# arangesh/Ground-Plane-Polling

Measured on AMD Instinct MI355X. Metric: images/sec end-to-end (resnet50, 1k planes, 1242x375), higher is better.
Workload: dtype f16x3

## Files before the change

ground-plane-polling_amd/csrc/decode.hip:

```cpp

#include <hip/hip_runtime.h>
#include <stdint.h>
#include <limits.h>

#include <atomic>
#include <mutex>
#include <vector>

#include "gpp.h"

namespace {

constexpr int kCounterStride = 4096;
constexpr int kHeaderBytes = 64 * kCounterStride;
constexpr int kKeptCountWord = 1;
constexpr int kKeptKeysOffset = 1024;

__device__ __forceinline__ float cephes_expf(float x)
{
    x = fminf(fmaxf(x, -88.3762626647949f), 88.3762626647949f);
    float fx = floorf(x * 1.44269504088896341f + 0.5f);
    x = (x - fx * 0.693359375f) - fx * -2.12194440e-4f;
    const float z = x * x;
    float y = 1.9875691500e-4f;
// ... 767 lines not shown
{
    compact_pixels(bitmap, T, B, max_rows, rows, counts, flag, or_flag);
}

struct CompactJob { uint32_t* bitmap; int32_t* rows; int32_t* counts; int32_t* flag; const int32_t* or_flag; };
__global__ __launch_bounds__(kCompactThreads) void compact_pixels_pair_kernel(const CompactJob a, const CompactJob b, const LevelTable T, int B, int max_rows)
{
    const CompactJob& j = blockIdx.x == 0 ? a : b;
    compact_pixels(j.bitmap, T, B, max_rows, j.rows, j.counts, j.flag, j.or_flag);
}

__global__ __launch_bounds__(256) void mark_candidate_pixels_kernel(const float* __restrict__ cls, int64_t n_anchors, int nba, float thr,
                                                                    const LevelTable T, int B, int total_words, uint32_t* __restrict__ marks)
{
    __shared__ unsigned long long hit[4];
    const int lane = threadIdx.x & 63, wave = threadIdx.x >> 6;
    const int64_t gbit0 = (int64_t)blockIdx.x * 256 + wave * 64;
    const int word0 = (int)(gbit0 >> 5);
    if (lane == 0) hit[wave] = 0;
    __syncthreads();
    for (int i = 0; i < nba; ++i) {
        const int j = i * 64 + lane, q = j / nba, k = j - q * nba;
        const int word = word0 + (q >> 5);
        if (word >= total_words) continue;
        int l = 0;
        for (int t = 1; t < T.n_levels; ++t) l = word >= T.word_begin[t] ? t : l;
        const int64_t bit = gbit0 + q - ((int64_t)T.word_begin[l] << 5);
        const int pix = T.pix[l];
        if (bit >= (int64_t)B * pix) continue;
        const int b = (int)(bit / pix), p = (int)(bit - (int64_t)b * pix);
        const float4* src = (const float4*)(cls + ((int64_t)b * n_anchors + (int64_t)(T.pix_begin[l] + p) * nba + k) * 8);
        const float4 v0 = src[0], v1 = src[1];
        const float lg[8] = {v0.x, v0.y, v0.z, v0.w, v1.x, v1.y, v1.z, v1.w};
        Folded f;
        if (is_candidate(lg, thr, f)) atomicOr(&hit[wave], 1ull << q);
    }
    __syncthreads();
    const unsigned long long mask = hit[wave];
    if (lane == 0 && word0 < total_words) marks[word0] = (uint32_t)mask;
    if (lane == 32 && word0 + 1 < total_words) marks[word0 + 1] = (uint32_t)(mask >> 32);
}

__global__ __launch_bounds__(256) void dilate_radii_kernel(const uint32_t* __restrict__ marks, const LevelTable T, int B, int total_words,
                                                           uint32_t* __restrict__ radius1, uint32_t* __restrict__ radius2,
                                                           uint32_t* __restrict__ radius3)
{
    const int64_t gbit = (int64_t)blockIdx.x * 256 + threadIdx.x;
    const int word = (int)(gbit >> 5);
    if (word >= total_words) return;
    int l = 0;
    for (int q = 1; q < T.n_levels; ++q) l = word >= T.word_begin[q] ? q : l;
    const int64_t bit = gbit - ((int64_t)T.word_begin[l] << 5);
    const int pix = T.pix[l], W = T.width[l], H = pix / W;
    bool on1 = false, on2 = false, on3 = false;
    if (bit < (int64_t)B * pix) {
        const int b = (int)(bit / pix), p = (int)(bit - (int64_t)b * pix);
        const int y = p / W, x = p - y * W;
        const uint32_t* words = marks + T.word_begin[l];
        for (int dy = -3; dy <= 3; ++dy) {
            const int yy = y + dy;
            if (yy < 0 || yy >= H) continue;
            for (int dx = -3; dx <= 3; ++dx) {
                const int xx = x + dx;
                if (xx < 0 || xx >= W) continue;
                const int64_t nb = (int64_t)b * pix + yy * W + xx;
                const bool v = (words[nb >> 5] >> (nb & 31)) & 1u;
                const int r = max(abs(dy), abs(dx));
                on3 |= v;
                on2 |= v && r <= 2;
                on1 |= v && r <= 1;
            }
        }
    }
    const unsigned long long m1 = __ballot(on1), m2 = __ballot(on2), m3 = __ballot(on3);
    const int lane = threadIdx.x & 63;
    if (lane == 0 || lane == 32) {
        const int sh = lane;
        radius1[word] = (uint32_t)(m1 >> sh);
        radius2[word] = (uint32_t)(m2 >> sh);
        radius3[word] = (uint32_t)(m3 >> sh);
    }
}

__global__ __launch_bounds__(kCompactThreads) void deep_stats_kernel(const uint32_t* __restrict__ marks, const uint32_t* __restrict__ radius1,
                                                                     const uint32_t* __restrict__ radius2, int total_words, int max_rows,
                                                                     int tower_max_rows, int deep_max_rows, int32_t* __restrict__ stats)
{
    __shared__ int sums[3][kCompactThreads / 64];
    const int tid = threadIdx.x, lane = tid & 63, wave = tid >> 6;
    int n[3] = {0, 0, 0};
    for (int w = tid; w < total_words; w += kCompactThreads) {
        n[0] += __popc(marks[w]);
        n[1] += __popc(radius1[w]);
        n[2] += __popc(radius2[w]);
    }
#pragma unroll
    for (int k = 0; k < 3; ++k) {
#pragma unroll
        for (int s = 32; s >= 1; s >>= 1) n[k] += __shfl_down(n[k], s, 64);
        if (lane == 0) sums[k][wave] = n[k];
    }
    __syncthreads();
    if (tid == 0) {
        int t[3] = {0, 0, 0};
        for (int q = 0; q < kCompactThreads / 64; ++q) { t[0] += sums[0][q]; t[1] += sums[1][q]; t[2] += sums[2][q]; }
        const int f3 = (t[0] > max_rows || t[1] > tower_max_rows) ? 1 : 0;
        stats[0] = t[0];
        stats[1] = t[1];
        stats[2] = f3;
        stats[3] = (f3 || t[2] > deep_max_rows) ? 1 : 0;
    }
}

std::mutex g_deep_mutex;
std::vector<gpp_deep_list_desc> g_deep_descs;
std::vector<char> g_deep_held;

}

extern "C" int gpp_detect_pixel_lists(const gpp_pixel_list_desc* host_desc, void* stream)
{
    if (!host_desc) return GPP_ERR_BAD_ARG;
    const gpp_pixel_list_desc& d = *host_desc;
    if (d.B < 0 || d.B > kMaxBatch || d.n_anchors <= 0 || d.n_anchors > kMaxAnchors || d.num_base_anchors <= 0 || d.max_rows < 0 ||
        d.n_levels < 1 || d.n_levels > GPP_MAX_GROUPS || (d.lists_per_image != 1 && d.lists_per_image != 4) || d.reserved != 0 || d.reserved2 != 0)
        return GPP_ERR_BAD_ARG;
    if (d.B == 0) return GPP_OK;
    if (!d.workspace || !d.bitmap || !d.rows || !d.counts || !d.flag) return GPP_ERR_BAD_ARG;
    if (((uintptr_t)d.workspace & 15) || (((uintptr_t)d.bitmap | (uintptr_t)d.rows | (uintptr_t)d.counts | (uintptr_t)d.flag) & 3)) return GPP_ERR_ALIGN;
    const bool dilate = d.dilated_bitmap || d.dilated_rows || d.dilated_counts || d.dilated_flag;
    if (dilate && (!d.dilated_bitmap || !d.dilated_rows || !d.dilated_counts || !d.dilated_flag || d.dilated_max_rows < 0)) return GPP_ERR_BAD_ARG;
    if (((uintptr_t)d.dilated_bitmap | (uintptr_t)d.dilated_rows | (uintptr_t)d.dilated_counts | (uintptr_t)d.dilated_flag) & 3) return GPP_ERR_ALIGN;
    const int lists = d.B * d.lists_per_image;
    if (lists > 64) return GPP_ERR_UNSUPPORTED;
    LevelTable T;
    T.n_levels = d.n_levels;
    int64_t pixels = 0, words = 0;
    for (int l = 0; l < GPP_MAX_GROUPS; ++l) {
        const int pix = l < d.n_levels ? d.level_pixels[l] : 0;
        if (l < d.n_levels && pix <= 0) return GPP_ERR_BAD_ARG;
        if ((int64_t)d.B * (pixels + pix) >= (1LL << 31)) return GPP_ERR_UNSUPPORTED;
        T.pix[l] = pix;
        T.pix_begin[l] = (int)pixels;
        T.word_begin[l] = (int)words;
        T.list_begin[l] = (int)((int64_t)d.B * pixels);
        T.width[l] = (dilate && l < d.n_levels) ? d.level_width[l] : 0;
        if (dilate && l < d.n_levels && (T.width[l] <= 0 || pix % T.width[l] != 0)) return GPP_ERR_BAD_ARG;
        pixels += pix;
        words += ((int64_t)d.B * pix + 31) / 32;
    }
    if (pixels * d.num_base_anchors != d.n_anchors) return GPP_ERR_BAD_ARG;
    hipStream_t st = (hipStream_t)stream;
    const unsigned char* ws = (const unsigned char*)d.workspace;
    const int32_t* cnt = (const int32_t*)ws;
    const unsigned long long* keys = (const unsigned long long*)(ws + kHeaderBytes);
    mark_pixels_kernel<<<dim3(16, (unsigned)lists), 256, 0, st>>>(keys, cnt, pow2_ceil(d.n_anchors), d.n_anchors, d.num_base_anchors,
                                                                   d.lists_per_image, T, d.bitmap);
    if (dilate) {
        const int64_t pairs = (words + 1) / 2;
        dilate_pixels_kernel<<<dim3((unsigned)((pairs * 64 + 255) / 256)), 256, 0, st>>>(d.bitmap, T, d.B, (int)words, d.dilated_bitmap);
    }
    compact_pixels_kernel<<<1, kCompactThreads, 0, st>>>(d.bitmap, T, d.B, d.max_rows, d.rows, d.counts, d.flag, nullptr);
    if (dilate)
        compact_pixels_kernel<<<1, kCompactThreads, 0, st>>>(d.dilated_bitmap, T, d.B, d.dilated_max_rows, d.dilated_rows, d.dilated_counts,
                                                             d.dilated_flag, d.flag);
    const hipError_t e = hipGetLastError();
    return e == hipSuccess ? GPP_OK : (int)e;
}

namespace {

int deep_lists_table(const gpp_deep_list_desc& d, LevelTable& T, int64_t& words)
{
    if (d.B < 0 || d.B > kMaxBatch || d.n_anchors <= 0 || d.n_anchors > kMaxAnchors || d.num_base_anchors <= 0 || d.num_base_anchors > 64 ||
        d.max_rows < 0 || d.tower_max_rows < 0 || d.deep_max_rows < 0 || d.n_levels < 1 || d.n_levels > GPP_MAX_GROUPS || d.reserved != 0 ||
        !(d.score_thr == d.score_thr))
        return GPP_ERR_BAD_ARG;
    const bool layer1 = d.rows1 || d.counts1 || d.flag1;
    if (d.B > 0 && (!d.cls_logits || !d.marks || !d.radius1 || !d.radius2 || !d.radius3 || !d.rows2 || !d.counts2 || !d.flag2 || !d.stats ||
                    (layer1 && (!d.rows1 || !d.counts1 || !d.flag1))))
        return GPP_ERR_BAD_ARG;
    if (((uintptr_t)d.cls_logits & 15) || (((uintptr_t)d.marks | (uintptr_t)d.radius1 | (uintptr_t)d.radius2 | (uintptr_t)d.radius3 | (uintptr_t)d.rows2 |
          (uintptr_t)d.counts2 | (uintptr_t)d.flag2 | (uintptr_t)d.rows1 | (uintptr_t)d.counts1 | (uintptr_t)d.flag1 | (uintptr_t)d.stats) & 3))
        return GPP_ERR_ALIGN;
    T.n_levels = d.n_levels;
    int64_t pixels = 0;
    words = 0;
    for (int l = 0; l < GPP_MAX_GROUPS; ++l) {
        const int pix = l < d.n_levels ? d.level_pixels[l] : 0;
        if (l < d.n_levels && pix <= 0) return GPP_ERR_BAD_ARG;
        if ((int64_t)d.B * (pixels + pix) >= (1LL << 31)) return GPP_ERR_UNSUPPORTED;
        T.pix[l] = pix;
        T.pix_begin[l] = (int)pixels;
        T.word_begin[l] = (int)words;
        T.list_begin[l] = (int)((int64_t)d.B * pixels);
        T.width[l] = l < d.n_levels ? d.level_width[l] : 0;
        if (l < d.n_levels && (T.width[l] <= 0 || pix % T.width[l] != 0)) return GPP_ERR_BAD_ARG;
        pixels += pix;
        words += ((int64_t)d.B * pix + 31) / 32;
    }
    if (pixels * d.num_base_anchors != d.n_anchors) return GPP_ERR_BAD_ARG;
    return GPP_OK;
}

}

extern "C" int gpp_detect_deep_lists(const gpp_deep_list_desc* host_desc, void* stream)
{
    if (!host_desc) return GPP_ERR_BAD_ARG;
    const gpp_deep_list_desc& d = *host_desc;
    LevelTable T;
    int64_t words = 0;
    const int rc = deep_lists_table(d, T, words);
    if (rc != GPP_OK) return rc;
    if (d.B == 0) return GPP_OK;
    hipStream_t st = (hipStream_t)stream;
    const unsigned blocks = (unsigned)(((words + 1) / 2 * 64 + 255) / 256);
    mark_candidate_pixels_kernel<<<dim3(blocks), 256, 0, st>>>(d.cls_logits, d.n_anchors, d.num_base_anchors, d.score_thr, T, d.B, (int)words, d.marks);
    dilate_radii_kernel<<<dim3(blocks), 256, 0, st>>>(d.marks, T, d.B, (int)words, d.radius1, d.radius2, d.radius3);
    deep_stats_kernel<<<1, kCompactThreads, 0, st>>>(d.marks, d.radius1, d.radius2, (int)words, d.max_rows, d.tower_max_rows, d.deep_max_rows, d.stats);
    const CompactJob layer2 = {d.radius2, d.rows2, d.counts2, d.flag2, d.stats + 2}, layer1 = {d.radius3, d.rows1, d.counts1, d.flag1, d.stats + 3};
    if (d.rows1) compact_pixels_pair_kernel<<<2, kCompactThreads, 0, st>>>(layer2, layer1, T, d.B, d.deep_max_rows);
    else compact_pixels_kernel<<<1, kCompactThreads, 0, st>>>(d.radius2, T, d.B, d.deep_max_rows, d.rows2, d.counts2, d.flag2, d.stats + 2);
    const hipError_t e = hipGetLastError();
    return e == hipSuccess ? GPP_OK : (int)e;
}

extern "C" int gpp_detect_deep_lists_register(const gpp_deep_list_desc* host_desc, int32_t* handle)
{
    if (!host_desc || !handle) return GPP_ERR_BAD_ARG;
    LevelTable T;
    int64_t words = 0;
    const int rc = deep_lists_table(*host_desc, T, words);
    if (rc != GPP_OK) return rc;
    std::lock_guard<std::mutex> lock(g_deep_mutex);
    size_t slot = 0;
    while (slot < g_deep_held.size() && g_deep_held[slot]) ++slot;
    if (slot >= (size_t)INT_MAX - 1) return GPP_ERR_UNSUPPORTED;
    if (slot == g_deep_held.size()) { g_deep_held.push_back(0); g_deep_descs.push_back(*host_desc); }
    g_deep_descs[slot] = *host_desc;
    g_deep_held[slot] = 1;
    *handle = (int32_t)slot + 1;
    return GPP_OK;
}

extern "C" int gpp_detect_deep_lists_release(int32_t handle)
{
    std::lock_guard<std::mutex> lock(g_deep_mutex);
    if (handle < 1 || (size_t)handle > g_deep_held.size() || !g_deep_held[(size_t)handle - 1]) return GPP_ERR_BAD_ARG;
    g_deep_held[(size_t)handle - 1] = 0;
    return GPP_OK;
}

extern "C" int gpp_detect_deep_lists_run(int32_t handle, int check_only, void* stream)
{
    gpp_deep_list_desc d;
    {
        std::lock_guard<std::mutex> lock(g_deep_mutex);
        if (handle < 1 || (size_t)handle > g_deep_held.size() || !g_deep_held[(size_t)handle - 1]) return GPP_ERR_BAD_ARG;
        d = g_deep_descs[(size_t)handle - 1];
    }
    return check_only ? GPP_OK : gpp_detect_deep_lists(&d, stream);
}

extern "C" int gpp_detect_workspace_bytes(int B, int64_t n_anchors, size_t* bytes)
{
    if (!bytes || B < 0 || B > kMaxBatch || n_anchors <= 0 || n_anchors > kMaxAnchors) return GPP_ERR_BAD_ARG;
    *bytes = detect_bytes(B, n_anchors, 1);
    return GPP_OK;
}

extern "C" int gpp_detect_osf_workspace_bytes(int B, int64_t n_anchors, size_t* bytes)
{
    if (!bytes || B < 0 || B > kMaxBatch || n_anchors <= 0 || n_anchors > kMaxAnchors) return GPP_ERR_BAD_ARG;
    *bytes = detect_bytes(B, n_anchors, 4);
    return GPP_OK;
}

extern "C" int gpp_detect_stages_f32(int stages, const float* cls_logits, const float* regression,
                                     const float* regression_dim, const float* anchors, int B, int64_t n_anchors,
                                     int num_base_anchors, int fused_layout, float score_thr, float iou_thr, int max_det,
                                     float* boxes, float* dims, float* scores, int32_t* labels, int32_t* orientations,
                                     int32_t* anchor_index, int32_t* counts,
                                     void* workspace, size_t workspace_bytes, void* stream)
{
    return detect_impl(stages, 1, cls_logits, regression, regression_dim, anchors, B, n_anchors, num_base_anchors, fused_layout, score_thr,
                       iou_thr, max_det, boxes, dims, scores, labels, orientations, anchor_index, counts, workspace, workspace_bytes, stream);
}

extern "C" int gpp_detect_osf_f32(const float* cls_logits, const float* regression, const float* regression_dim,
                                  const float* anchors, int B, int64_t n_anchors, int num_base_anchors, int fused_layout,
                                  float score_thr, float iou_thr, int max_det,
                                  float* boxes, float* dims, float* scores, int32_t* labels, int32_t* orientations,
                                  int32_t* anchor_index, int32_t* counts,
                                  void* workspace, size_t workspace_bytes, void* stream)
{
    return detect_impl(GPP_DETECT_CANDIDATES | GPP_DETECT_SELECT | GPP_DETECT_EMIT, 4, cls_logits, regression, regression_dim, anchors, B,
                       n_anchors, num_base_anchors, fused_layout, score_thr, iou_thr, max_det, boxes, dims, scores, labels, orientations,
                       anchor_index, counts, workspace, workspace_bytes, stream);
}

extern "C" int gpp_detect_f32(const float* cls_logits, const float* regression, const float* regression_dim,
                              const float* anchors, int B, int64_t n_anchors, int num_base_anchors, int fused_layout,
                              float score_thr, float iou_thr, int max_det,
                              float* boxes, float* dims, float* scores, int32_t* labels, int32_t* orientations,
                              int32_t* anchor_index, int32_t* counts,
                              void* workspace, size_t workspace_bytes, void* stream)
{
    return gpp_detect_stages_f32(GPP_DETECT_CANDIDATES | GPP_DETECT_SELECT | GPP_DETECT_EMIT, cls_logits, regression, regression_dim,
                                 anchors, B, n_anchors, num_base_anchors, fused_layout, score_thr, iou_thr, max_det, boxes, dims,
                                 scores, labels, orientations, anchor_index, counts, workspace, workspace_bytes, stream);
}
```

ground-plane-polling_amd/keras_retinanet_3D/backend/hip.py:

```python

import ctypes
import os

_LIB = None
_HERE = os.path.dirname(os.path.abspath(__file__))
LIB_PATH = os.environ.get('GPP_LIB') or os.path.normpath(os.path.join(_HERE, '..', '..', 'lib', 'libgpp_hip.so'))
CSRC_DIR = os.path.normpath(os.path.join(_HERE, '..', '..', 'csrc'))

GPP_OK = 0
_ERRORS = {
    -1: 'GPP_ERR_BAD_ARG',
    -2: 'GPP_ERR_WORKSPACE',
    -3: 'GPP_ERR_ALIGN',
    -4: 'GPP_ERR_UNSUPPORTED',
}

c_void_p = ctypes.c_void_p
c_int = ctypes.c_int
c_float = ctypes.c_float
c_size_t = ctypes.c_size_t
c_int64 = ctypes.c_int64


GPP_BF16 = 1
GPP_F16 = 2
GPP_F32 = 3
GPP_BF16X3 = 4
GPP_F16X3 = 5
GPP_MAX_GROUPS = 5
GPP_DRAW_PRIM_WORDS = 16
GPP_DRAW_PRIMS_PER_DET = 26
GPP_DRAW_COUNT_WORDS = 4
GPP_POSE_COLS = 36
GPP_EVAL_MAX_DETECTIONS, GPP_EVAL_MAX_ANNOTATIONS = 1024, 1024
GPP_EVAL_ANN_COLS, GPP_EVAL_ERR_COLS = 17, 11
GPP_KITTI_MAX_DETECTIONS, GPP_KITTI_MAX_LABELS = 128, 128
GPP_KITTI_MAX_THRESHOLDS, GPP_KITTI_LABEL_COLS = 41, 16
GPP_LABEL_MOD_COLS = 20
GPP_ABSMAX_F32, GPP_ABSMAX_SPLIT_F16, GPP_ABSMAX_SPLIT_BF16 = 1, 2, 3


class GppError(RuntimeError):
    pass


class ConvGroup(ctypes.Structure):
    _fields_ = [('in_off', c_int64), ('in_bstride', c_int64), ('out_off', c_int64), ('out_bstride', c_int64),
                ('res_off', c_int64), ('res_bstride', c_int64),
                ('H_in', ctypes.c_int32), ('W_in', ctypes.c_int32), ('H_out', ctypes.c_int32), ('W_out', ctypes.c_int32),
                ('H_res', ctypes.c_int32), ('W_res', ctypes.c_int32), ('tile_start', ctypes.c_int32),
                ('row_begin', ctypes.c_int32)]


class ConvDesc(ctypes.Structure):
    _fields_ = [('inp', c_void_p), ('weight', c_void_p), ('bias', c_void_p), ('residual', c_void_p),
                ('out', c_void_p), ('zero_page', c_void_p),
                ('dtype', ctypes.c_int32), ('out_f32', ctypes.c_int32),
                ('batch', ctypes.c_int32), ('C_in', ctypes.c_int32), ('C_out', ctypes.c_int32),
                ('KH', ctypes.c_int32), ('KW', ctypes.c_int32), ('stride', ctypes.c_int32),
                ('pad_top', ctypes.c_int32), ('pad_left', ctypes.c_int32),
                ('in_pitch', ctypes.c_int32), ('out_pitch', ctypes.c_int32), ('res_pitch', ctypes.c_int32),
                ('weight_rows', ctypes.c_int32), ('relu', ctypes.c_int32), ('n_groups', ctypes.c_int32),
                ('tile_hint', ctypes.c_int32), ('reserved', ctypes.c_int32),
                ('in_bytes', ctypes.c_int32), ('weight_bytes', ctypes.c_int32),
                ('partial', c_void_p), ('partial_bytes', c_int64), ('split_k', ctypes.c_int32), ('partial_rows', ctypes.c_int32),
                ('groups', ConvGroup * GPP_MAX_GROUPS),
                ('x3_split', ctypes.c_int32), ('reserved2', ctypes.c_int32), ('out_scale', c_void_p), ('range_counter', c_void_p),
                ('gather_rows', c_void_p), ('gather_counts', c_void_p), ('guard', c_void_p),
                ('guard_value', ctypes.c_int32), ('reserved3', ctypes.c_int32),
                ('tower_rows', c_void_p), ('tower_counts', c_void_p), ('tower_flag', c_void_p),
                ('tower_tile', ctypes.c_int32), ('reserved4', ctypes.c_int32),
                ('deep_rows', c_void_p), ('deep_counts', c_void_p), ('deep_flag', c_void_p),
                ('deep_tile', ctypes.c_int32), ('lists_after', ctypes.c_int32)]


class PixelListDesc(ctypes.Structure):
    _fields_ = [('workspace', c_void_p), ('bitmap', c_void_p), ('rows', c_void_p), ('counts', c_void_p), ('flag', c_void_p),
                ('n_anchors', c_int64)] + \
               [(n, ctypes.c_int32) for n in ('B', 'num_base_anchors', 'lists_per_image', 'n_levels', 'max_rows', 'reserved')] + \
               [('level_pixels', ctypes.c_int32 * GPP_MAX_GROUPS), ('reserved2', ctypes.c_int32)] + \
               [('dilated_bitmap', c_void_p), ('dilated_rows', c_void_p), ('dilated_counts', c_void_p), ('dilated_flag', c_void_p),
                ('level_width', ctypes.c_int32 * GPP_MAX_GROUPS), ('dilated_max_rows', ctypes.c_int32)]


class DeepListDesc(ctypes.Structure):
    _fields_ = [(n, c_void_p) for n in ('cls_logits', 'marks', 'radius1', 'radius2', 'radius3', 'rows2', 'counts2', 'flag2',
                                        'rows1', 'counts1', 'flag1', 'stats')] + [('n_anchors', c_int64)] + \
               [(n, ctypes.c_int32) for n in ('B', 'num_base_anchors', 'n_levels', 'max_rows', 'tower_max_rows', 'deep_max_rows')] + \
               [('score_thr', c_float), ('reserved', ctypes.c_int32),
                ('level_pixels', ctypes.c_int32 * GPP_MAX_GROUPS), ('level_width', ctypes.c_int32 * GPP_MAX_GROUPS)]


class MobileNetBlockDesc(ctypes.Structure):
    _fields_ = [('inp', c_void_p), ('dw_weight', c_void_p), ('dw_bias', c_void_p), ('pw_weight', c_void_p), ('pw_bias', c_void_p),
                ('out_scale', c_void_p), ('out', c_void_p)] + \
               [(n, ctypes.c_int32) for n in ('dtype', 'B', 'H', 'W', 'C_in', 'C_out', 'stride', 'in_pitch', 'out_pitch', 'weight_rows',
                                              'tile_hint', 'reserved')]


class MobileNetStemDesc(ctypes.Structure):
    _fields_ = [('inp', c_void_p), ('weight', c_void_p), ('bias', c_void_p), ('out', c_void_p)] + \
               [(n, ctypes.c_int32) for n in ('B', 'H', 'W', 'C_out', 'out_pitch', 'reserved')]


class AbsmaxDesc(ctypes.Structure):
    _fields_ = [('inp', c_void_p), ('out', c_void_p), ('M', c_int64), ('pitch', c_int64)] + \
               [(n, ctypes.c_int32) for n in ('C', 'c_off', 'layout', 'reserved')]


class AbsmaxClearDesc(ctypes.Structure):
    _fields_ = [('table', c_void_p), ('n', c_int64)]


def _declare(lib):
    lib.gpp_version.restype = ctypes.c_char_p
    lib.gpp_version.argtypes = []
    lib.gpp_poll_workspace_bytes.restype = c_int
    lib.gpp_poll_workspace_bytes.argtypes = [c_int, c_int, c_int, ctypes.POINTER(c_size_t)]
    lib.gpp_poll_f32.restype = c_int
    lib.gpp_poll_f32.argtypes = [c_void_p] * 5 + [c_int, c_int, c_int, c_int, c_float] + [c_void_p] * 4 + \
        [c_void_p, c_size_t, c_void_p]
    lib.gpp_pose_f32.restype = c_int
    lib.gpp_pose_f32.argtypes = [c_void_p] * 8 + [c_int, c_int, c_float] + [c_void_p] * 3
    if hasattr(lib, 'gpp_draw_build'):
        lib.gpp_draw_workspace_bytes.restype = c_int
        lib.gpp_draw_workspace_bytes.argtypes = [c_int, c_int, ctypes.POINTER(c_size_t), ctypes.POINTER(c_size_t)]
        lib.gpp_draw_build.restype = c_int
        lib.gpp_draw_build.argtypes = [c_void_p, c_void_p, c_int, c_int, c_float, c_void_p, c_void_p, c_void_p]
        lib.gpp_draw_raster.restype = c_int
        lib.gpp_draw_raster.argtypes = [c_void_p, c_void_p, c_int, c_int, c_void_p, c_void_p, c_int, c_void_p, c_void_p, c_void_p]
    if hasattr(lib, 'gpp_eval_match_f32'):
        lib.gpp_eval_match_f32.restype = c_int
        lib.gpp_eval_match_f32.argtypes = [c_void_p] * 8 + [c_int] * 4 + [c_float, c_int, ctypes.c_double] + [c_void_p] * 4
    if hasattr(lib, 'gpp_kitti_overlaps_f64'):
        lib.gpp_kitti_overlaps_f64.restype = c_int
        lib.gpp_kitti_overlaps_f64.argtypes = [c_void_p] * 3 + [c_int] * 3 + [c_void_p] * 2
        lib.gpp_kitti_stats_f64.restype = c_int
        lib.gpp_kitti_stats_f64.argtypes = [c_void_p] * 4 + [ctypes.POINTER(ctypes.c_double)] + [c_void_p] * 2 + [c_int] * 4 + [c_void_p] * 5
    if hasattr(lib, 'gpp_label_prep_f64'):
        lib.gpp_label_prep_f64.restype = c_int
        lib.gpp_label_prep_f64.argtypes = [c_void_p] * 4 + [c_int, c_int, ctypes.c_uint, c_int] + [c_void_p] * 7
    if hasattr(lib, 'gpp_poll_costs_u16'):
        lib.gpp_poll_costs_workspace_bytes.restype = c_int
        lib.gpp_poll_costs_workspace_bytes.argtypes = [c_int, ctypes.POINTER(c_size_t)]
        lib.gpp_poll_costs_u16.restype = c_int
        lib.gpp_poll_costs_u16.argtypes = [c_void_p] * 5 + [c_int, c_int, c_int, c_float, c_void_p, c_int, c_void_p, c_int64, c_int64,
                                           c_void_p, c_size_t, c_void_p]
        lib.gpp_plane_select_workspace_bytes.restype = c_int
        lib.gpp_plane_select_workspace_bytes.argtypes = [c_int, ctypes.POINTER(c_size_t)]
        lib.gpp_plane_select.restype = c_int
        lib.gpp_plane_select.argtypes = [c_void_p, c_int, c_int, c_int64, c_int] + [c_void_p] * 4 + [c_void_p, c_size_t, c_void_p]
    if hasattr(lib, 'gpp_detect_pixel_lists'):
        lib.gpp_detect_pixel_lists.restype = c_int
        lib.gpp_detect_pixel_lists.argtypes = [ctypes.POINTER(PixelListDesc), c_void_p]
    if hasattr(lib, 'gpp_detect_deep_lists'):
        lib.gpp_detect_deep_lists.restype = c_int
        lib.gpp_detect_deep_lists.argtypes = [ctypes.POINTER(DeepListDesc), c_void_p]
        lib.gpp_detect_deep_lists_register.restype = c_int
        lib.gpp_detect_deep_lists_register.argtypes = [ctypes.POINTER(DeepListDesc), ctypes.POINTER(ctypes.c_int32)]
        lib.gpp_detect_deep_lists_release.restype = c_int
        lib.gpp_detect_deep_lists_release.argtypes = [ctypes.c_int32]
        lib.gpp_detect_deep_lists_run.restype = c_int
        lib.gpp_detect_deep_lists_run.argtypes = [ctypes.c_int32, c_int, c_void_p]
    lib.gpp_conv2d_igemm.restype = c_int
    lib.gpp_conv2d_igemm.argtypes = [ctypes.POINTER(ConvDesc), c_void_p]
    lib.gpp_stem_conv7x7_bn_relu.restype = c_int
    lib.gpp_stem_conv7x7_bn_relu.argtypes = [c_void_p, c_void_p, c_void_p, c_void_p, c_int, c_int, c_int, c_int, c_void_p]
    lib.gpp_stem_conv7x7_bn_relu_mfma.restype = c_int
    lib.gpp_stem_conv7x7_bn_relu_mfma.argtypes = [c_void_p, c_void_p, c_void_p, c_void_p, c_int, c_int, c_int, c_int, c_void_p]
    lib.gpp_stem_pack_weights_f16.restype = c_int
    lib.gpp_stem_pack_weights_f16.argtypes = [c_void_p, c_void_p, c_size_t]
    lib.gpp_stem_pack_weights_f16x3.restype = c_int
    lib.gpp_stem_pack_weights_f16x3.argtypes = [c_void_p, c_void_p, c_size_t]
# ... 331 lines not shown
```

ground-plane-polling_amd/keras_retinanet_3D/models/plan.py:

```python

import collections
import ctypes

import numpy as np

from ..backend import hip
from ..layers import conv as C


class StemDesc(ctypes.Structure):
    _fields_ = [('inp', ctypes.c_void_p), ('weight', ctypes.c_void_p), ('bias', ctypes.c_void_p), ('out', ctypes.c_void_p),
                ('dtype', ctypes.c_int32), ('B', ctypes.c_int32), ('H', ctypes.c_int32), ('W', ctypes.c_int32), ('range_counter', ctypes.c_void_p)]


class PoolDesc(ctypes.Structure):
    _fields_ = [('inp', ctypes.c_void_p), ('out', ctypes.c_void_p), ('dtype', ctypes.c_int32), ('B', ctypes.c_int32),
                ('H', ctypes.c_int32), ('W', ctypes.c_int32), ('C', ctypes.c_int32), ('reserved', ctypes.c_int32)]


class RaggedStemDesc(ctypes.Structure):
    _fields_ = [('stem', StemDesc), ('heights', ctypes.c_void_p), ('Hp', ctypes.c_int32), ('reserved', ctypes.c_int32)]


class RaggedPoolDesc(ctypes.Structure):
# ... 64 lines not shown
OP_DETECT_CANDIDATE_PIXELS = 40
DETECT_OPS = (OP_DETECT, OP_DETECT_CANDIDATES, OP_DETECT_SELECT, OP_DETECT_EMIT, 12, OP_DETECT_CANDIDATE_PIXELS)
OP_JOIN, OP_SYNC = 0x10000, 0x20000


PlanOptions = collections.namedtuple('PlanOptions', 'x3_level fuse_stem_pool stage_chunks half_stages fuse_tail fuse_block fuse_block_proj '
                                                    'br1_lane fpn_lanes p4_lane head_lanes decode_overlap cls_lane autotune tune_key sparse_heads '
                                                    'sparse_tower sparse_tower_rounds sparse_deep sparse_deep_rounds sparse_depth')


def block_form(opts, width, projection, split_input, halves, join):
    if width in opts.fuse_block and (not projection or opts.fuse_block_proj) and split_input:
        launch = 'block'
    else:
        launch = 'tail' if width in opts.fuse_tail else 'convs'
    if not projection:
        return launch, 'identity'
    return launch, 'side' if opts.br1_lane and not halves and not join else 'inline'


def part_of(fm, c0, nb):
    return C.FMap(fm.buf, nb, fm.H, fm.W, fm.C, off=fm.off + c0 * fm.bstride, bstride=fm.bstride, pitch=fm.pitch, split=fm.split, half=fm.half)


TOWER_SLICES = {('pyramid_towers_0', 0): 'pyramid_regression_0', ('pyramid_towers_0', 512): 'pyramid_classification_0',
                ('pyramid_towers_0', 768): 'pyramid_regression_dim_0'}
RANGE_AUDIT_THRESHOLD = 2.0 ** -9
X3_QUANTUM = 2.0 ** -24
SPARSE_HEADS_MAX_SHARE = '0.5'
SPARSE_TOWER_MAX_SHARE = '0.75'
SPARSE_TOWER_MIN_ROUNDS = '1'
SPARSE_TOWER_DEPTH = '3'
SPARSE_TOWER_DEEP_MAX_SHARE = '0.75'
SPARSE_TOWER_DEEP_MIN_ROUNDS = '1'
COMPUTE_UNITS = 256


def audit_report(maps, table, threshold=RANGE_AUDIT_THRESHOLD):
    table = np.ascontiguousarray(table).view(np.uint32).reshape(-1)
    out = []
    for m in maps:
        first, n = m['row']
        bits = table[first:first + n]
        vals = bits.view(np.float32).astype(np.float64)
        live = vals[bits != 0]
        finite = live[~np.isnan(live)]
        absmax = float('nan') if len(finite) < len(live) else float(finite.max()) if len(finite) else 0.0
        rec = {k: m[k] for k in ('name', 'consumers', 'channels') if k in m}
        rec.update({'live': int(len(live)), 'absmax': absmax,
                    'absmax_min_live': float(finite.min()) if len(finite) else None,
                    'absmax_median_live': float(np.median(finite)) if len(finite) else None,
                    'small_channels': int((finite < threshold).sum()),
                    'bits': None if not absmax > 0 else int(min(22, max(0, np.floor(np.log2(absmax / X3_QUANTUM))))) if np.isfinite(absmax) else 22,
                    'flagged': bool(0 < absmax < threshold)})
        out.append(rec)
    return out


class SparseHeads(object):

    def __init__(self, torch, device, B, level_pixels, max_share, level_widths=None, tower_share=0.0):
        i32 = torch.int32
        self.B, self.level_pixels = B, [int(p) for p in level_pixels]
        self.level_widths = [int(w) for w in level_widths] if level_widths else []
        total = B * sum(self.level_pixels)
        self.max_rows = max(0, min(total, int(max_share * total)))
        self.bitmap = torch.zeros((sum((B * p + 31) // 32 for p in self.level_pixels),), dtype=i32, device=device)
        self.rows = torch.zeros((total,), dtype=i32, device=device)
        self.counts = torch.zeros((hip.GPP_MAX_GROUPS + 1,), dtype=i32, device=device)
        self.flag = torch.ones((1,), dtype=i32, device=device)
        self.dense, self.gathered = [], []
        self.lists_joined = False
        self.tower, self.tower_max_rows = [], 0
        self.tower_bitmap = self.tower_rows = self.tower_counts = self.tower_flag = self.range_scratch = None
        if tower_share > 0.0:
            self.tower_max_rows = max(0, min(total, int(tower_share * total)))
            self.tower_bitmap = torch.zeros_like(self.bitmap)
            self.tower_rows = torch.zeros_like(self.rows)
            self.tower_counts = torch.zeros_like(self.counts)
            self.tower_flag = torch.ones_like(self.flag)
            self.range_scratch = torch.zeros((1,), dtype=torch.int64, device=device)

        self.deep, self.deep_layers, self.deep_max_rows, self.deep_handle = [], 0, 0, 0
        self.deep_bitmaps = self.deep_rows = self.deep_counts = self.deep_flags = self.deep_stats = None

    def add_deep(self, torch, layers, deep_share):
        total = self.B * sum(self.level_pixels)
        self.deep_layers = int(layers)
        self.deep_max_rows = max(0, min(total, int(deep_share * total)))
        self.deep_bitmaps = [torch.zeros_like(self.bitmap) for _ in range(4)]
        self.deep_rows = [torch.zeros_like(self.rows) for _ in range(self.deep_layers)]
        self.deep_counts = [torch.zeros_like(self.counts) for _ in range(self.deep_layers)]
        self.deep_flags = [torch.ones_like(self.flag) for _ in range(self.deep_layers)]
        self.deep_stats = torch.zeros((4,), dtype=torch.int32, device=self.rows.device)

    def deep_tensors(self):
        if self.deep_rows is None:
            return []
        return self.deep_bitmaps + self.deep_rows + self.deep_counts + self.deep_flags + [self.deep_stats]

    def deep_desc(self, cls_logits, n_anchors, num_base_anchors, score_thr):
        d = hip.DeepListDesc()
        d.cls_logits = cls_logits.data_ptr()
        d.marks, d.radius1, d.radius2, d.radius3 = [t.data_ptr() for t in self.deep_bitmaps]
        d.rows2, d.counts2, d.flag2 = self.deep_rows[0].data_ptr(), self.deep_counts[0].data_ptr(), self.deep_flags[0].data_ptr()
        if self.deep_layers > 1:
            d.rows1, d.counts1, d.flag1 = self.deep_rows[1].data_ptr(), self.deep_counts[1].data_ptr(), self.deep_flags[1].data_ptr()
        d.stats = self.deep_stats.data_ptr()
        d.n_anchors, d.B, d.num_base_anchors, d.n_levels = n_anchors, self.B, num_base_anchors, len(self.level_pixels)
        d.max_rows, d.tower_max_rows, d.deep_max_rows, d.score_thr = self.max_rows, self.tower_max_rows, self.deep_max_rows, score_thr
        d.level_pixels = (ctypes.c_int32 * hip.GPP_MAX_GROUPS)(*self.level_pixels)
        d.level_width = (ctypes.c_int32 * hip.GPP_MAX_GROUPS)(*self.level_widths)
        return d

    def register_deep(self, desc):
        handle = ctypes.c_int32(0)
        hip.check(hip.lib().gpp_detect_deep_lists_register(ctypes.byref(desc), ctypes.byref(handle)), 'gpp_detect_deep_lists_register')
        self.deep_handle = int(handle.value)
        return self.deep_handle

    def __del__(self):
        if getattr(self, 'deep_handle', 0):
            try:
                hip.lib().gpp_detect_deep_lists_release(self.deep_handle)
            except Exception:
                pass
            self.deep_handle = 0

    def tensors(self):
        own = [self.bitmap, self.rows, self.counts, self.flag]
        return own + ([self.tower_bitmap, self.tower_rows, self.tower_counts, self.tower_flag] if self.tower_rows is not None else [])

    def put_every_nth(self, torch, n=8, tower=False):
        rows, cnt = (self.tower_rows, self.tower_counts) if tower else (self.rows, self.counts)
        begin, counts = 0, []
        for p in self.level_pixels:
            idx = torch.arange(0, self.B * p, n, dtype=torch.int32, device=rows.device)
            rows[begin:begin + idx.numel()] = idx
            counts.append(int(idx.numel()))
            begin += self.B * p
        counts += [0] * (hip.GPP_MAX_GROUPS - len(counts)) + [sum(counts)]
        cnt.copy_(torch.as_tensor(counts, dtype=torch.int32))

    def reset(self, torch):
        self.counts.zero_()
        self.flag.fill_(1)
        if self.tower_rows is not None:
            self.tower_counts.zero_()
            self.tower_flag.fill_(1)
        self.reset_deep()

    def reset_deep(self):
        for flag in self.deep_flags or ():
            flag.fill_(1)


class Plan(object):

    def __init__(self):
        self.keep = []
        self.io = {}
        self.io_parts = {}
        self.tuning_parts = {}
        self.ops = []
        self.oracle_names = {}
        self.lanes = []
        self.access = []
        self.atomic = []
        self.wrote = []
        self.op_io = []
        self.audit_table = None
        self.audit_maps = []
        self.audit_unobserved = []
        self.inner = {}
        self.open_lanes = set()
        self.conv_descs = []
        self.ws_need = {}
        self.array = None
        self.flops = 0.0
        self.ragged = False
        self.heights = None
        self.sparse = None
        self.heads_stale = False

    @property
    def regression(self):
        self.complete_heads()
        return self._regression

    @regression.setter
    def regression(self, tensor):
# ... 141 lines not shown
```

include/gpp.h:

```cpp
#ifndef GPP_H_
#define GPP_H_

#include <stddef.h>
#include <stdint.h>

#ifdef __cplusplus
extern "C" {
#endif

#define GPP_OK 0
#define GPP_ERR_BAD_ARG (-1)
#define GPP_ERR_WORKSPACE (-2)
#define GPP_ERR_ALIGN (-3)
#define GPP_ERR_UNSUPPORTED (-4)

const char* gpp_version(void);

int gpp_poll_workspace_bytes(int B, int N, int planes_batched, size_t* bytes);

int gpp_poll_f32(const float* boxes, const float* dims, const int32_t* orient, const float* P_inv,
                 const float* planes, int B, int D, int N, int planes_batched, float thr,
                 float* keypoints, float* keyplanes, float* residuals, int32_t* best_idx,
                 void* workspace, size_t workspace_bytes, void* stream);

// ... 100 lines not shown
int gpp_mobilenet_block_autotune(gpp_mobilenet_block_desc* desc, int iters, void* stream, float* best_us);
int gpp_mobilenet_stem(const float* in, const float* weight, const float* bias, float* out, int B, int H, int W, int C_out, int out_pitch,
                       void* stream);
int gpp_mobilenet_depthwise(const float* in, const float* weight, const float* bias, float* out, int B, int H, int W, int C, int stride,
                            int in_pitch, int out_pitch, void* stream);

int gpp_stem_conv7x7_bn_relu(const float* in, const float* weight, const float* bias, void* out, int dtype,
                             int B, int H, int W, void* stream);
int gpp_stem_pack_weights_f16(const float* host_weight_147x64, void* host_packed, size_t packed_bytes);
int gpp_stem_conv7x7_bn_relu_mfma(const float* in, const void* packed_weight_f16, const float* bias, void* out,
                                  int dtype, int B, int H, int W, void* stream);
int gpp_maxpool3x3s2_same(const void* in, void* out, int dtype, int B, int H, int W, int C, void* stream);
int gpp_stem_pool_fused_mfma(const float* in, const void* packed_weight_f16, const float* bias, void* out,
                             int dtype, int B, int H, int W, void* stream);
int gpp_stem_pack_weights_f16x3(const float* host_weight_147x64, void* host_packed, size_t packed_bytes);
int gpp_stem_conv7x7_bn_relu_x3(const float* in, const void* packed_weight_x3, const float* bias, float* out,
                                int B, int H, int W, void* stream);
int gpp_stem_conv7x7_bn_relu_x3_rc(const float* in, const void* packed_weight_x3, const float* bias, float* out,
                                   int B, int H, int W, uint64_t* range_counter, void* stream);
int gpp_stem_pool_fused_x3(const float* in, const void* packed_weight_x3, const float* bias, float* out,
                           int B, int H, int W, uint64_t* range_counter, void* stream);
int gpp_stem_conv7x7_bn_relu_ragged(const float* in, const float* weight, const float* bias, void* out, int dtype,
                                    int B, int H, int W, int Hp, const int32_t* heights, void* stream);
int gpp_stem_conv7x7_bn_relu_mfma_ragged(const float* in, const void* packed_weight_f16, const float* bias, void* out,
                                         int dtype, int B, int H, int W, int Hp, const int32_t* heights, void* stream);
int gpp_stem_conv7x7_bn_relu_x3_rc_ragged(const float* in, const void* packed_weight_x3, const float* bias, float* out,
                                          int B, int H, int W, int Hp, const int32_t* heights, uint64_t* range_counter, void* stream);
int gpp_maxpool3x3s2_same_ragged(const void* in, void* out, int dtype, int B, int H, int W, int C, int Hp,
                                 const int32_t* heights, void* stream);
int gpp_stem_pool_fused_mfma_ragged(const float* in, const void* packed_weight_f16, const float* bias, void* out,
                                    int dtype, int B, int H, int W, int Hp, const int32_t* heights, void* stream);
int gpp_stem_pool_fused_x3_ragged(const float* in, const void* packed_weight_x3, const float* bias, float* out,
                                  int B, int H, int W, int Hp, const int32_t* heights, uint64_t* range_counter, void* stream);
int gpp_relu(const void* in, void* out, int dtype, int64_t count, void* stream);
int gpp_relu_strided(const void* in, int64_t in_bstride, void* out, int64_t out_bstride, int dtype, int B,
                     int64_t count, void* stream);

int gpp_preprocess_u8_bgr(const uint8_t* frames, float* out, const int32_t* y0, const int32_t* y1, const float* wy,
                          const int32_t* x0, const int32_t* x1, const float* wx, int B, int H, int W, int Ho, int Wo,
                          float mean_b, float mean_g, float mean_r, void* stream);
int gpp_preprocess_u8_bgr_ragged(const uint8_t* frames, float* out, const int32_t* raw_hw, const int32_t* heights,
                                 const int32_t* y0, const int32_t* y1, const float* wy, const int32_t* x0, const int32_t* x1, const float* wx,
                                 int B, int H, int W, int Hp, int Ho, int Wo, float mean_b, float mean_g, float mean_r, void* stream);

int gpp_detect_workspace_bytes(int B, int64_t n_anchors, size_t* bytes);

int gpp_detect_f32(const float* cls_logits, const float* regression, const float* regression_dim,
                   const float* anchors, int B, int64_t n_anchors, int num_base_anchors, int fused_layout,
                   float score_thr, float iou_thr, int max_det,
                   float* boxes, float* dims, float* scores, int32_t* labels, int32_t* orientations,
                   int32_t* anchor_index, int32_t* counts,
                   void* workspace, size_t workspace_bytes, void* stream);

#define GPP_DETECT_CANDIDATES 1
#define GPP_DETECT_SELECT 2
#define GPP_DETECT_EMIT 4
int gpp_detect_stages_f32(int stages, const float* cls_logits, const float* regression, const float* regression_dim,
                          const float* anchors, int B, int64_t n_anchors, int num_base_anchors, int fused_layout,
                          float score_thr, float iou_thr, int max_det,
                          float* boxes, float* dims, float* scores, int32_t* labels, int32_t* orientations,
                          int32_t* anchor_index, int32_t* counts,
                          void* workspace, size_t workspace_bytes, void* stream);

typedef struct gpp_pixel_list_desc {
    const void* workspace; uint32_t* bitmap; int32_t* rows; int32_t* counts; int32_t* flag;
    int64_t n_anchors;
    int32_t B, num_base_anchors, lists_per_image, n_levels, max_rows, reserved;
    int32_t level_pixels[GPP_MAX_GROUPS]; int32_t reserved2;
    uint32_t* dilated_bitmap; int32_t* dilated_rows; int32_t* dilated_counts; int32_t* dilated_flag;
    int32_t level_width[GPP_MAX_GROUPS]; int32_t dilated_max_rows;
} gpp_pixel_list_desc;
int gpp_detect_pixel_lists(const gpp_pixel_list_desc* host_desc, void* stream);

typedef struct gpp_deep_list_desc {
    const float* cls_logits;
    uint32_t* marks; uint32_t* radius1; uint32_t* radius2; uint32_t* radius3;
    int32_t* rows2; int32_t* counts2; int32_t* flag2;
    int32_t* rows1; int32_t* counts1; int32_t* flag1;
    int32_t* stats;
    int64_t n_anchors;
    int32_t B, num_base_anchors, n_levels, max_rows, tower_max_rows, deep_max_rows;
    float score_thr; int32_t reserved;
    int32_t level_pixels[GPP_MAX_GROUPS]; int32_t level_width[GPP_MAX_GROUPS];
} gpp_deep_list_desc;
int gpp_detect_deep_lists(const gpp_deep_list_desc* host_desc, void* stream);
int gpp_detect_deep_lists_register(const gpp_deep_list_desc* host_desc, int32_t* handle);
int gpp_detect_deep_lists_release(int32_t handle);
int gpp_detect_deep_lists_run(int32_t handle, int check_only, void* stream);

int gpp_detect_osf_workspace_bytes(int B, int64_t n_anchors, size_t* bytes);
int gpp_detect_osf_f32(const float* cls_logits, const float* regression, const float* regression_dim,
                       const float* anchors, int B, int64_t n_anchors, int num_base_anchors, int fused_layout,
                       float score_thr, float iou_thr, int max_det,
                       float* boxes, float* dims, float* scores, int32_t* labels, int32_t* orientations,
                       int32_t* anchor_index, int32_t* counts,
                       void* workspace, size_t workspace_bytes, void* stream);

int gpp_pack_detections(const float* boxes, const float* dims, const float* scores, const int32_t* labels,
                        const int32_t* orientations, const float* keypoints, const float* keyplanes,
                        const float* residuals, int B, int D, float* packed, void* stream);

#define GPP_POSE_COLS 36
int gpp_pose_f32(const float* boxes, const float* dims, const float* scores, const int32_t* labels,
                 const int32_t* orientations, const float* keypoints, const float* residuals,
                 const float* frame_info, int B, int D, float score_thr,
                 float* rows, int32_t* counts, void* stream);

#define GPP_EVAL_MAX_DETECTIONS 1024
#define GPP_EVAL_MAX_ANNOTATIONS 1024
#define GPP_EVAL_ANN_COLS 17
#define GPP_EVAL_ERR_COLS 11
int gpp_eval_match_f32(const float* boxes, const float* dims, const float* scores, const int32_t* labels,
                       const int32_t* orientations, const float* scales, const double* annotations,
                       const int32_t* ann_counts, int B, int D, int A, int num_classes, float score_thr,
                       int max_detections, double iou_thr, int32_t* table, double* errors, int32_t* counts, void* stream);

#define GPP_KITTI_MAX_DETECTIONS 128
#define GPP_KITTI_MAX_LABELS 128
#define GPP_KITTI_MAX_THRESHOLDS 41
#define GPP_KITTI_LABEL_COLS 16
int gpp_kitti_overlaps_f64(const float* rows, const double* labels, const int32_t* label_counts, int B, int D, int A,
                           double* overlaps, void* stream);
int gpp_kitti_stats_f64(const float* rows, const double* labels, const int32_t* label_counts, const double* overlaps,
                        const double* min_overlap, const float* thresholds, const int32_t* n_thresholds, int B, int D, int A, int T,
                        float* tp_scores, int32_t* n_gt, int32_t* stats, double* similarity, void* stream);

#define GPP_LABEL_MOD_COLS 20
int gpp_label_prep_f64(const double* labels, const int32_t* label_counts, const double* P, const double* trig, int B, int A,
                       unsigned det_types, int own_box, double* mod,
                       float* boxes, float* dims, float* scores, int32_t* det_labels, int32_t* orientations, void* stream);

#define GPP_PLANE_COST_INVALID 65535
int gpp_poll_costs_workspace_bytes(int M, size_t* bytes);
int gpp_poll_costs_u16(const float* boxes, const float* dims, const int32_t* orient, const float* P_inv, const float* planes,
                       int B, int D, int M, float thr, const int32_t* row_index, int O, uint16_t* table, int64_t pitch,
                       int64_t row_offset, void* workspace, size_t workspace_bytes, void* stream);
int gpp_plane_select_workspace_bytes(int M, size_t* bytes);
int gpp_plane_select(const uint16_t* table, int O, int M, int64_t pitch, int K, int32_t* chosen, uint64_t* trace,
                     uint16_t* best, int32_t* count, void* workspace, size_t workspace_bytes, void* stream);

#define GPP_DRAW_PRIM_WORDS 16
#define GPP_DRAW_PRIMS_PER_DET 26
#define GPP_DRAW_COUNT_WORDS 4
#define GPP_DRAW_CAPTION_MAX 20
#define GPP_DRAW_NONE 0
#define GPP_DRAW_LINE 1
#define GPP_DRAW_DASHED 2
#define GPP_DRAW_RECT 3
#define GPP_DRAW_CIRCLE 4
#define GPP_DRAW_CAPTION 5
int gpp_draw_workspace_bytes(int B, int D, size_t* prims_bytes, size_t* workspace_bytes);
int gpp_draw_build(const float* rows, const double* P, int B, int D, float score_thr, void* prims, int32_t* counts, void* stream);
int gpp_draw_raster(const uint8_t* frames_u8, const int32_t* raw_hw, int Hr, int Wr, const void* prims, const int32_t* counts,
                    int B, uint8_t* out_u8, void* workspace, void* stream);

#define GPP_ABSMAX_F32 1
#define GPP_ABSMAX_SPLIT_F16 2
#define GPP_ABSMAX_SPLIT_BF16 3
typedef struct gpp_absmax_desc {
    const void* in; uint32_t* out;
    int64_t M, pitch;
    int32_t C, c_off, layout, reserved;
} gpp_absmax_desc;
typedef struct gpp_absmax_clear_desc { uint32_t* table; int64_t n; } gpp_absmax_clear_desc;
int gpp_channel_absmax(const gpp_absmax_desc* desc, void* stream);
int gpp_absmax_clear(uint32_t* table, int64_t n, void* stream);

// ... 91 lines not shown
```

Baseline: 911.2.

## Parallelize deep pixel-list compaction across chunked blocks with per-chunk prefix offsets

Replaces the single-block compaction of the deep dilation bitmaps with a two-phase scheme. The stats kernel now also computes per-64-word chunk popcounts and scans them per level into base offsets, counts and overflow flags. A new multi-block kernel then writes row indices per chunk in parallel and clears the bitmap words. This removes the serial one-block compaction bottleneck, at the cost of an extra scratch buffer, an ABI change to the descriptor, and a serial per-level scan done by one wave per layer.

```diff
diff --git a/ground-plane-polling_amd/csrc/decode.hip b/ground-plane-polling_amd/csrc/decode.hip
--- a/ground-plane-polling_amd/csrc/decode.hip
+++ b/ground-plane-polling_amd/csrc/decode.hip
@@ -873,17 +873,65 @@
     }
 }
 
+__device__ __forceinline__ int level_chunks(const LevelTable& T, int B, int l)
+{
+    return (((B * T.pix[l] + 31) >> 5) + GPP_DEEP_CHUNK_WORDS - 1) / GPP_DEEP_CHUNK_WORDS;
+}
+
+__device__ __forceinline__ void chunk_words(const LevelTable& T, int B, int c, int& l, int& first, int& end)
+{
+    l = 0;
+    int begin = 0;
+    for (int q = 0; q + 1 < T.n_levels; ++q) {
+        const int next = begin + level_chunks(T, B, q);
+        if (c < next) break;
+        l = q + 1;
+        begin = next;
+    }
+    first = T.word_begin[l] + (c - begin) * GPP_DEEP_CHUNK_WORDS;
+    end = T.word_begin[l] + ((B * T.pix[l] + 31) >> 5);
+}
+
+__device__ __forceinline__ int wave_inclusive_scan(int v, int lane)
+{
+#pragma unroll
+    for (int s = 1; s < 64; s <<= 1) {
+        const int up = __shfl_up(v, s, 64);
+        if (lane >= s) v += up;
+    }
+    return v;
+}
+
+struct DeepListOut { int32_t* counts; int32_t* flag; };
 __global__ __launch_bounds__(kCompactThreads) void deep_stats_kernel(const uint32_t* __restrict__ marks, const uint32_t* __restrict__ radius1,
-                                                                     const uint32_t* __restrict__ radius2, int total_words, int max_rows,
-                                                                     int tower_max_rows, int deep_max_rows, int32_t* __restrict__ stats)
+                                                                     const uint32_t* __restrict__ radius2, const uint32_t* __restrict__ radius3,
+                                                                     const LevelTable T, int B, int n_chunks, int max_rows, int tower_max_rows,
+                                                                     int deep_max_rows, int32_t* __restrict__ stats, int32_t* chunk_base,
+                                                                     const DeepListOut out2, const DeepListOut out1)
 {
     __shared__ int sums[3][kCompactThreads / 64];
     const int tid = threadIdx.x, lane = tid & 63, wave = tid >> 6;
     int n[3] = {0, 0, 0};
-    for (int w = tid; w < total_words; w += kCompactThreads) {
-        n[0] += __popc(marks[w]);
-        n[1] += __popc(radius1[w]);
-        n[2] += __popc(radius2[w]);
+    for (int c = wave; c < n_chunks; c += kCompactThreads / 64) {
+        int l, first, end;
+        chunk_words(T, B, c, l, first, end);
+        const int w = first + lane;
+        int c2 = 0, c3 = 0;
+        if (w < end) {
+            n[0] += __popc(marks[w]);
+            n[1] += __popc(radius1[w]);
+            c2 = __popc(radius2[w]);
+            if (radius3 != nullptr) c3 = __popc(radius3[w]);
+        }
+        n[2] += c2;
+        if (chunk_base != nullptr) {
+#pragma unroll
+            for (int s = 32; s >= 1; s >>= 1) { c2 += __shfl_down(c2, s, 64); c3 += __shfl_down(c3, s, 64); }
+            if (lane == 0) {
+                chunk_base[c] = c2;
+                if (radius3 != nullptr) chunk_base[n_chunks + c] = c3;
+            }
+        }
     }
 #pragma unroll
     for (int k = 0; k < 3; ++k) {
@@ -891,15 +939,66 @@
         for (int s = 32; s >= 1; s >>= 1) n[k] += __shfl_down(n[k], s, 64);
         if (lane == 0) sums[k][wave] = n[k];
     }
+    __threadfence();
     __syncthreads();
+    int t[3] = {0, 0, 0};
+    for (int q = 0; q < kCompactThreads / 64; ++q) { t[0] += sums[0][q]; t[1] += sums[1][q]; t[2] += sums[2][q]; }
+    const int f3 = (t[0] > max_rows || t[1] > tower_max_rows) ? 1 : 0;
+    const int f2 = (f3 || t[2] > deep_max_rows) ? 1 : 0;
     if (tid == 0) {
-        int t[3] = {0, 0, 0};
-        for (int q = 0; q < kCompactThreads / 64; ++q) { t[0] += sums[0][q]; t[1] += sums[1][q]; t[2] += sums[2][q]; }
-        const int f3 = (t[0] > max_rows || t[1] > tower_max_rows) ? 1 : 0;
         stats[0] = t[0];
         stats[1] = t[1];
         stats[2] = f3;
-        stats[3] = (f3 || t[2] > deep_max_rows) ? 1 : 0;
+        stats[3] = f2;
+    }
+    if (chunk_base == nullptr || wave > (radius3 != nullptr ? 1 : 0)) return;
+    volatile int32_t* base = chunk_base + (wave ? n_chunks : 0);
+    const DeepListOut& out = wave ? out1 : out2;
+    int total = 0, level_begin = 0;
+    for (int l = 0; l < GPP_MAX_GROUPS; ++l) {
+        int running = 0;
+        if (l < T.n_levels) {
+            const int nc = level_chunks(T, B, l);
+            for (int c0 = 0; c0 < nc; c0 += 64) {
+                const int c = c0 + lane;
+                const int v = c < nc ? base[level_begin + c] : 0;
+                const int incl = wave_inclusive_scan(v, lane);
+                if (c < nc) base[level_begin + c] = running + incl - v;
+                running += __shfl(incl, 63, 64);
+            }
+            level_begin += nc;
+        }
+        if (lane == 0) out.counts[l] = running;
+        total += running;
+    }
+    if (lane == 0) {
+        out.counts[GPP_MAX_GROUPS] = total;
+        out.flag[0] = (total > deep_max_rows || (wave ? f2 : f3)) ? 1 : 0;
+    }
+}
+
+struct ChunkJob { uint32_t* bitmap; int32_t* rows; };
+__global__ __launch_bounds__(64) void compact_chunks_kernel(const ChunkJob a, const ChunkJob b, const int32_t* __restrict__ chunk_base, int n_chunks,
+                                                            const LevelTable T, int B)
+{
+    const ChunkJob& j = blockIdx.y == 0 ? a : b;
+    const int c = blockIdx.x, lane = threadIdx.x;
+    int l, first, end;
+    chunk_words(T, B, c, l, first, end);
+    const int w = first + lane;
+    uint32_t word = 0;
+    if (w < end) {
+        word = j.bitmap[w];
+        if (word) j.bitmap[w] = 0;
+    }
+    const int n = __popc(word);
+    int pos = chunk_base[blockIdx.y * n_chunks + c] + wave_inclusive_scan(n, lane) - n;
+    const int bit0 = (w - T.word_begin[l]) * 32, capacity = B * T.pix[l];
+    while (word) {
+        const int bit = __ffs((int)word) - 1;
+        word &= word - 1;
+        if (pos >= 0 && pos < capacity) j.rows[T.list_begin[l] + pos] = bit0 + bit;
+        ++pos;
     }
 }
 
@@ -961,7 +1060,7 @@
 
 namespace {
 
-int deep_lists_table(const gpp_deep_list_desc& d, LevelTable& T, int64_t& words)
+int deep_lists_table(const gpp_deep_list_desc& d, LevelTable& T, int64_t& words, int64_t& chunks)
 {
     if (d.B < 0 || d.B > kMaxBatch || d.n_anchors <= 0 || d.n_anchors > kMaxAnchors || d.num_base_anchors <= 0 || d.num_base_anchors > 64 ||
         d.max_rows < 0 || d.tower_max_rows < 0 || d.deep_max_rows < 0 || d.n_levels < 1 || d.n_levels > GPP_MAX_GROUPS || d.reserved != 0 ||
@@ -972,7 +1071,8 @@
                     (layer1 && (!d.rows1 || !d.counts1 || !d.flag1))))
         return GPP_ERR_BAD_ARG;
     if (((uintptr_t)d.cls_logits & 15) || (((uintptr_t)d.marks | (uintptr_t)d.radius1 | (uintptr_t)d.radius2 | (uintptr_t)d.radius3 | (uintptr_t)d.rows2 |
-          (uintptr_t)d.counts2 | (uintptr_t)d.flag2 | (uintptr_t)d.rows1 | (uintptr_t)d.counts1 | (uintptr_t)d.flag1 | (uintptr_t)d.stats) & 3))
+          (uintptr_t)d.counts2 | (uintptr_t)d.flag2 | (uintptr_t)d.rows1 | (uintptr_t)d.counts1 | (uintptr_t)d.flag1 | (uintptr_t)d.stats |
+          (uintptr_t)d.chunk_base) & 3))
         return GPP_ERR_ALIGN;
     T.n_levels = d.n_levels;
     int64_t pixels = 0;
@@ -991,6 +1091,9 @@
         words += ((int64_t)d.B * pix + 31) / 32;
     }
     if (pixels * d.num_base_anchors != d.n_anchors) return GPP_ERR_BAD_ARG;
+    chunks = 0;
+    for (int l = 0; l < d.n_levels; ++l) chunks += (((int64_t)d.B * d.level_pixels[l] + 31) / 32 + GPP_DEEP_CHUNK_WORDS - 1) / GPP_DEEP_CHUNK_WORDS;
+    if (d.chunk_base ? d.chunk_base_ints < 2 * chunks : d.chunk_base_ints != 0) return GPP_ERR_BAD_ARG;
     return GPP_OK;
 }
 
@@ -1001,18 +1104,25 @@
     if (!host_desc) return GPP_ERR_BAD_ARG;
     const gpp_deep_list_desc& d = *host_desc;
     LevelTable T;
-    int64_t words = 0;
-    const int rc = deep_lists_table(d, T, words);
+    int64_t words = 0, n_chunks = 0;
+    const int rc = deep_lists_table(d, T, words, n_chunks);
     if (rc != GPP_OK) return rc;
     if (d.B == 0) return GPP_OK;
     hipStream_t st = (hipStream_t)stream;
     const unsigned blocks = (unsigned)(((words + 1) / 2 * 64 + 255) / 256);
     mark_candidate_pixels_kernel<<<dim3(blocks), 256, 0, st>>>(d.cls_logits, d.n_anchors, d.num_base_anchors, d.score_thr, T, d.B, (int)words, d.marks);
     dilate_radii_kernel<<<dim3(blocks), 256, 0, st>>>(d.marks, T, d.B, (int)words, d.radius1, d.radius2, d.radius3);
-    deep_stats_kernel<<<1, kCompactThreads, 0, st>>>(d.marks, d.radius1, d.radius2, (int)words, d.max_rows, d.tower_max_rows, d.deep_max_rows, d.stats);
-    const CompactJob layer2 = {d.radius2, d.rows2, d.counts2, d.flag2, d.stats + 2}, layer1 = {d.radius3, d.rows1, d.counts1, d.flag1, d.stats + 3};
-    if (d.rows1) compact_pixels_pair_kernel<<<2, kCompactThreads, 0, st>>>(layer2, layer1, T, d.B, d.deep_max_rows);
-    else compact_pixels_kernel<<<1, kCompactThreads, 0, st>>>(d.radius2, T, d.B, d.deep_max_rows, d.rows2, d.counts2, d.flag2, d.stats + 2);
+    const DeepListOut out2 = {d.counts2, d.flag2}, out1 = {d.counts1, d.flag1};
+    deep_stats_kernel<<<1, kCompactThreads, 0, st>>>(d.marks, d.radius1, d.radius2, d.rows1 ? d.radius3 : nullptr, T, d.B, (int)n_chunks, d.max_rows,
+                                                     d.tower_max_rows, d.deep_max_rows, d.stats, d.chunk_base, out2, out1);
+    if (d.chunk_base) {
+        const ChunkJob layer2 = {d.radius2, d.rows2}, layer1 = {d.radius3, d.rows1};
+        compact_chunks_kernel<<<dim3((unsigned)n_chunks, d.rows1 ? 2 : 1), 64, 0, st>>>(layer2, layer1, d.chunk_base, (int)n_chunks, T, d.B);
+    } else {
+        const CompactJob layer2 = {d.radius2, d.rows2, d.counts2, d.flag2, d.stats + 2}, layer1 = {d.radius3, d.rows1, d.counts1, d.flag1, d.stats + 3};
+        if (d.rows1) compact_pixels_pair_kernel<<<2, kCompactThreads, 0, st>>>(layer2, layer1, T, d.B, d.deep_max_rows);
+        else compact_pixels_kernel<<<1, kCompactThreads, 0, st>>>(d.radius2, T, d.B, d.deep_max_rows, d.rows2, d.counts2, d.flag2, d.stats + 2);
+    }
     const hipError_t e = hipGetLastError();
     return e == hipSuccess ? GPP_OK : (int)e;
 }
@@ -1021,8 +1131,8 @@
 {
     if (!host_desc || !handle) return GPP_ERR_BAD_ARG;
     LevelTable T;
-    int64_t words = 0;
-    const int rc = deep_lists_table(*host_desc, T, words);
+    int64_t words = 0, chunks = 0;
+    const int rc = deep_lists_table(*host_desc, T, words, chunks);
     if (rc != GPP_OK) return rc;
     std::lock_guard<std::mutex> lock(g_deep_mutex);
     size_t slot = 0;
diff --git a/ground-plane-polling_amd/keras_retinanet_3D/backend/hip.py b/ground-plane-polling_amd/keras_retinanet_3D/backend/hip.py
--- a/ground-plane-polling_amd/keras_retinanet_3D/backend/hip.py
+++ b/ground-plane-polling_amd/keras_retinanet_3D/backend/hip.py
@@ -28,6 +28,7 @@
 GPP_BF16X3 = 4
 GPP_F16X3 = 5
 GPP_MAX_GROUPS = 5
+GPP_DEEP_CHUNK_WORDS = 64
 GPP_DRAW_PRIM_WORDS = 16
 GPP_DRAW_PRIMS_PER_DET = 26
 GPP_DRAW_COUNT_WORDS = 4
@@ -88,7 +89,8 @@
                                         'rows1', 'counts1', 'flag1', 'stats')] + [('n_anchors', c_int64)] + \
                [(n, ctypes.c_int32) for n in ('B', 'num_base_anchors', 'n_levels', 'max_rows', 'tower_max_rows', 'deep_max_rows')] + \
                [('score_thr', c_float), ('reserved', ctypes.c_int32),
-                ('level_pixels', ctypes.c_int32 * GPP_MAX_GROUPS), ('level_width', ctypes.c_int32 * GPP_MAX_GROUPS)]
+                ('level_pixels', ctypes.c_int32 * GPP_MAX_GROUPS), ('level_width', ctypes.c_int32 * GPP_MAX_GROUPS),
+                ('chunk_base', c_void_p), ('chunk_base_ints', c_int64)]
 
 
 class MobileNetBlockDesc(ctypes.Structure):
diff --git a/ground-plane-polling_amd/keras_retinanet_3D/models/plan.py b/ground-plane-polling_amd/keras_retinanet_3D/models/plan.py
--- a/ground-plane-polling_amd/keras_retinanet_3D/models/plan.py
+++ b/ground-plane-polling_amd/keras_retinanet_3D/models/plan.py
@@ -170,7 +170,7 @@
             self.range_scratch = torch.zeros((1,), dtype=torch.int64, device=device)
 
         self.deep, self.deep_layers, self.deep_max_rows, self.deep_handle = [], 0, 0, 0
-        self.deep_bitmaps = self.deep_rows = self.deep_counts = self.deep_flags = self.deep_stats = None
+        self.deep_bitmaps = self.deep_rows = self.deep_counts = self.deep_flags = self.deep_stats = self.deep_chunk_base = None
 
     def add_deep(self, torch, layers, deep_share):
         total = self.B * sum(self.level_pixels)
@@ -181,11 +181,13 @@
         self.deep_counts = [torch.zeros_like(self.counts) for _ in range(self.deep_layers)]
         self.deep_flags = [torch.ones_like(self.flag) for _ in range(self.deep_layers)]
         self.deep_stats = torch.zeros((4,), dtype=torch.int32, device=self.rows.device)
+        chunks = sum(-(-((self.B * p + 31) // 32) // hip.GPP_DEEP_CHUNK_WORDS) for p in self.level_pixels)
+        self.deep_chunk_base = torch.zeros((2 * chunks,), dtype=torch.int32, device=self.rows.device)
 
     def deep_tensors(self):
         if self.deep_rows is None:
             return []
-        return self.deep_bitmaps + self.deep_rows + self.deep_counts + self.deep_flags + [self.deep_stats]
+        return self.deep_bitmaps + self.deep_rows + self.deep_counts + self.deep_flags + [self.deep_stats, self.deep_chunk_base]
 
     def deep_desc(self, cls_logits, n_anchors, num_base_anchors, score_thr):
         d = hip.DeepListDesc()
@@ -195,6 +197,7 @@
         if self.deep_layers > 1:
             d.rows1, d.counts1, d.flag1 = self.deep_rows[1].data_ptr(), self.deep_counts[1].data_ptr(), self.deep_flags[1].data_ptr()
         d.stats = self.deep_stats.data_ptr()
+        d.chunk_base, d.chunk_base_ints = self.deep_chunk_base.data_ptr(), self.deep_chunk_base.numel()
         d.n_anchors, d.B, d.num_base_anchors, d.n_levels = n_anchors, self.B, num_base_anchors, len(self.level_pixels)
         d.max_rows, d.tower_max_rows, d.deep_max_rows, d.score_thr = self.max_rows, self.tower_max_rows, self.deep_max_rows, score_thr
         d.level_pixels = (ctypes.c_int32 * hip.GPP_MAX_GROUPS)(*self.level_pixels)
diff --git a/include/gpp.h b/include/gpp.h
--- a/include/gpp.h
+++ b/include/gpp.h
@@ -206,7 +206,9 @@
     int32_t B, num_base_anchors, n_levels, max_rows, tower_max_rows, deep_max_rows;
     float score_thr; int32_t reserved;
     int32_t level_pixels[GPP_MAX_GROUPS]; int32_t level_width[GPP_MAX_GROUPS];
+    int32_t* chunk_base; int64_t chunk_base_ints;
 } gpp_deep_list_desc;
+#define GPP_DEEP_CHUNK_WORDS 64
 int gpp_detect_deep_lists(const gpp_deep_list_desc* host_desc, void* stream);
 int gpp_detect_deep_lists_register(const gpp_deep_list_desc* host_desc, int32_t* handle);
 int gpp_detect_deep_lists_release(int32_t handle);
```

Result: no change. 911.8, median of 2 (+0.1%).
